# ChengeLi/LongTerm360FoV

Measured on AMD Instinct MI355X. Metric: sequences/sec (batch=1024, T_in=30->T_out=30, h=256), higher is better.
Workload: dtype f32; 1 GPU; configs[1]: target-only seq2seq inference (encoder + autoregressive decoder), H=256, batch=1024 per GPU, T_in=30->T_out=30, F_enc=90, F_dec=6, fp32, act=sigmoid, impl=auto; global_batch=1024, parallelism=replicas x1 (no collective)

## Files before the change

include/fov360.h:

```cpp
#ifndef FOV360_H
#define FOV360_H

#include <stddef.h>
#include <stdint.h>

#ifdef __cplusplus
extern "C" {
#endif

typedef void* fov_stream_t;

enum { FOV_ACT_SIGMOID = 0, FOV_ACT_HARD_SIGMOID = 1 };

enum {
    FOV_IMPL_AUTO = 0,
    FOV_IMPL_GENERIC = 1,
    FOV_IMPL_CLUSTER = 2
};

enum {
    FOV_OK = 0,
    FOV_ERR_INVALID = -1,
    FOV_ERR_UNSUPPORTED = -2,
    FOV_ERR_WORKSPACE = -3,
// ... 147 lines not shown
int fov_lstm_seq_fwd_zx(const float* zx, const float* R, const float* b, const float* h0, const float* c0,
                        float* hs, float* hT, float* cT, float* reserve,
                        int B, int T, int H, int act, int impl,
                        void* workspace, size_t workspace_bytes, fov_stream_t stream);

size_t fov_seq2seq_decode_workspace_bytes(int B, int T_in, int T_out, int F_enc, int F_dec, int H, int impl);
int fov_seq2seq_decode_fwd(const float* enc_in, const float* dec_in0,
                           const float* enc_K, const float* enc_R, const float* enc_b,
                           const float* dec_K, const float* dec_R, const float* dec_b,
                           const float* dense_W, const float* dense_b,
                           float* out, float* hT, float* cT,
                           int B, int T_in, int T_out, int F_enc, int F_dec, int H,
                           int act, int impl,
                           void* workspace, size_t workspace_bytes, fov_stream_t stream);

int fov_seq2seq_decoder_fwd(const float* dec_in0, const float* h0, const float* c0, const float* dec_K,
                            const float* dec_R, const float* dec_b, const float* dense_W, const float* dense_b,
                            float* out, float* hT, float* cT, int B, int T_out, int F_dec, int H, int act, int impl,
                            void* workspace, size_t workspace_bytes, fov_stream_t stream);

int fov_stacked_seq2seq_decode_supported(int B, int T_in, int T_out, int F_enc, int F_dec, int H, int L);
int fov_stacked_seq2seq_decode_fwd(const float* enc_in, const float* dec_in0,
                                   const float* enc0_K, const float* enc0_R, const float* enc0_b,
                                   const float* enc1_K, const float* enc1_R, const float* enc1_b,
                                   const float* enc2_K, const float* enc2_R, const float* enc2_b,
                                   const float* dec0_K, const float* dec0_R, const float* dec0_b,
                                   const float* dec1_K, const float* dec1_R, const float* dec1_b,
                                   const float* dec2_K, const float* dec2_R, const float* dec2_b,
                                   const float* dense_W, const float* dense_b,
                                   float* out, float* hT, float* cT,
// ... 249 lines not shown
```

longterm360fov_amd/_lib.py:

```python
import ctypes
import os

_HERE = os.path.dirname(os.path.abspath(__file__))
LIB_PATH = os.environ.get("FOV_LIB_PATH") or os.path.join(_HERE, "lib", "libfov360_hip.so")

ACT_SIGMOID = 0
ACT_HARD_SIGMOID = 1
IMPL_AUTO = 0
IMPL_GENERIC = 1
IMPL_CLUSTER = 2

OK = 0
ERR_INVALID = -1
ERR_UNSUPPORTED = -2
ERR_WORKSPACE = -3
ERR_LAUNCH = -4
ERR_TIMEOUT = -5

_P = ctypes.c_void_p
_I = ctypes.c_int
_SZ = ctypes.c_size_t

SIGNATURES = {
    "fov_last_error": (ctypes.c_char_p, []),
# ... 7 lines not shown
    "fov_mix_head_bwd": (_I, [_P] * 9 + [_I] * 3 + [_P]),
    "fov_mix_decoder_workspace_bytes": (_SZ, [_I] * 2),
    "fov_mix_decoder_fwd": (_I, [_P] * 6 + [ctypes.c_int64] * 2 + [_P] * 21 + [_I] * 5 + [_P, _SZ, _P]),
    "fov_mix_decoder_fwd_bf16": (_I, [_P] * 6 + [ctypes.c_int64] * 2 + [_P] * 21 + [_I] * 5 + [_P, _SZ, _P]),
    "fov_lstm_seq_fwd_bf16": (_I, [_P] * 10 + [_I] * 5 + [_P, _SZ, _P]),
    "fov_seq2seq_decode_fwd_bf16": (_I, [_P] * 13 + [_I] * 7 + [_P, _SZ, _P]),
    "fov_dense_fwd_bf16": (_I, [_P] * 4 + [_I] * 4 + [_P]),
    "fov_mix_decoder_bwd_workspace_bytes": (_SZ, [_I] * 2),
    "fov_mix_decoder_bwd": (_I, [_P] * 21 + [_I] * 5 + [_P, _SZ, _P]),
    "fov_mix_decoder_bwd_bf16": (_I, [_P] * 21 + [_I] * 5 + [_P, _SZ, _P]),
    "fov_matmul_workspace_bytes": (_SZ, [_I] * 3),
    "fov_matmul": (_I, [_P] * 3 + [_I] * 3 + [_P, _SZ, _P]),
    "fov_lstm_seq_fwd_zx": (_I, [_P] * 9 + [_I] * 5 + [_P, _SZ, _P]),
    "fov_seq2seq_decode_workspace_bytes": (_SZ, [_I] * 7),
    "fov_seq2seq_decode_fwd": (_I, [_P] * 13 + [_I] * 8 + [_P, _SZ, _P]),
    "fov_seq2seq_decoder_fwd": (_I, [_P] * 11 + [_I] * 6 + [_P, _SZ, _P]),
    "fov_stacked_seq2seq_decode_supported": (_I, [_I] * 7),
    "fov_stacked_seq2seq_decode_fwd": (_I, [_P] * 25 + [_I] * 8 + [_P]),
    "fov_selffed_decoder_supported": (_I, [_I] * 4),
    "fov_selffed_decoder_fwd": (_I, [_P] * 15 + [_I] * 6 + [_P]),
    "fov_selffed_decoder_bwd": (_I, [_P] * 14 + [_I] * 7 + [_P]),
    "fov_stacked_seq2seq_train_supported": (_I, [_I] * 7),
    "fov_stacked_seq2seq_train_bwd_scratch_bytes": (_SZ, [_I] * 4),
    "fov_stacked_seq2seq_train_fwd": (_I, [_P] * 15 + [_I] * 8 + [_P]),
    "fov_stacked_seq2seq_train_bwd": (_I, [_P] * 10 + [_I] * 6 + [_P, _SZ, _P]),
    "fov_seq2seq_tf_workspace_bytes": (_SZ, [_I] * 7),
    "fov_seq2seq_tf_fwd": (_I, [_P] * 11 + [_I] * 8 + [_P, _SZ, _P]),
    "fov_meanvar_xyz": (_I, [_P, _P, ctypes.c_int64, _I, _P]),
    "fov_lstm_seq_fwd_train": (_I, [_P] * 10 + [_I] * 6 + [_P, _SZ, _P]),
    "fov_lstm_seq_bwd_workspace_bytes": (_SZ, [_I] * 4),
# ... 127 lines not shown
```

longterm360fov_amd/csrc/api_lstm.hip:

```cpp
#include "fov_common.h"
#include "xch_common.h"
#include "bf16_common.h"

namespace fov {

static bool want_cluster(int impl, int F, int H, int F_dec, bool decode) {
    if (impl == FOV_IMPL_GENERIC) return false;
    const bool ok = cluster_shape_ok(F, H) && (!decode || (F_dec >= 1 && F_dec <= 8)) && device_cu_count() >= H / 64;
    return impl == FOV_IMPL_CLUSTER ? true : ok;
}

static LstmParams layer_params(const float* x, const float* K, const float* R, const float* b, const float* h0, const float* c0,
                               float* hs, float* hT, float* cT, float* reserve, int B, int T, int F, int H, int act, void* workspace) {
    LstmParams p = {};
    p.x = x; p.K = K; p.R = R; p.b = b; p.h0 = h0; p.c0 = c0; p.hs = hs; p.hT = hT; p.cT = cT; p.reserve = reserve;
    p.B = B; p.T = T; p.F = F; p.H = H; p.act = act;
    bind_workspace(p, workspace);
    return p;
}

enum class FwdKernel { Wide16, Wide512, Wide, Cluster, Stepwise, Generic };
struct FwdPlan {
    FwdKernel kernel;
    size_t need;
// ... 400 lines not shown

int fov_mix_decoder_bwd_bf16(const float* M, const float* P, const float* dloss, const float* res1, const float* res2,
                             const float* C1, const float* C2, const float* dec1_K, const float* dec1_R, const float* dec2_K,
                             const float* dec2_R, const float* dense_W, const float* mix_Wp, float* DZ1, float* DZ2,
                             float* dpre_m, float* dpre_p, float* dh1_0, float* dc1_0, float* dh2_0, float* dc2_0, int B,
                             int T_out, int H, int O, int act, void* workspace, size_t workspace_bytes, fov_stream_t stream) {
    return mix_decoder_bwd_impl(M, P, dloss, res1, res2, C1, C2, dec1_K, dec1_R, dec2_K, dec2_R, dense_W, mix_Wp, DZ1, DZ2, dpre_m,
                                dpre_p, dh1_0, dc1_0, dh2_0, dc2_0, B, T_out, H, O, act, workspace, workspace_bytes, stream, true);
}

size_t fov_seq2seq_decode_workspace_bytes(int B, int T_in, int T_out, int F_enc, int F_dec, int H, int impl) {
    (void)T_in;
    return plan_decode(B, T_out, F_enc, F_dec, H, impl).need;
}

int fov_seq2seq_decode_fwd(const float* enc_in, const float* dec_in0, const float* enc_K, const float* enc_R,
                           const float* enc_b, const float* dec_K, const float* dec_R, const float* dec_b,
                           const float* dense_W, const float* dense_b, float* out, float* hT, float* cT, int B,
                           int T_in, int T_out, int F_enc, int F_dec, int H, int act, int impl, void* workspace,
                           size_t workspace_bytes, fov_stream_t stream) {
    if (B < 0 || T_in < 0 || T_out < 0 || F_enc <= 0 || F_dec <= 0 || H <= 0 || !enc_K || !enc_R || !enc_b ||
        !dec_K || !dec_R || !dec_b || !dense_W || !dense_b ||
        (B > 0 && ((T_in > 0 && !enc_in) || !dec_in0 || (T_out > 0 && !out))) || !valid_act(act)) {
        set_error("fov_seq2seq_decode_fwd: invalid argument");
        return FOV_ERR_INVALID;
    }
    if (F_dec > 64) { set_error("fov_seq2seq_decode_fwd: F_dec > 64 unsupported"); return FOV_ERR_UNSUPPORTED; }
    const DecodePlan plan = plan_decode(B, T_out, F_enc, F_dec, H, impl);
    if (int rc = check_ws(workspace, workspace_bytes, plan.need)) return rc;
    LstmParams p = {};
    p.x = enc_in; p.K = enc_K; p.R = enc_R; p.b = enc_b; p.T = T_in; p.F = F_enc;
    bind_decoder(p, dec_in0, dec_K, dec_R, dec_b, dense_W, dense_b, out, hT, cT, B, T_out, F_dec, H, act, workspace);
    hipStream_t s = (hipStream_t)stream;
    switch (plan.kernel) {
        case DecodeKernel::Wide16: return launch_wide16_s2s(p, s);
        case DecodeKernel::Cluster: return launch_cluster(p, true, s);
        case DecodeKernel::Generic: break;
    }
    return launch_generic(p, true, s);
}

int fov_seq2seq_decoder_fwd(const float* dec_in0, const float* h0, const float* c0, const float* dec_K,
                            const float* dec_R, const float* dec_b, const float* dense_W, const float* dense_b, float* out,
                            float* hT, float* cT, int B, int T_out, int F_dec, int H, int act, int impl, void* workspace,
                            size_t workspace_bytes, fov_stream_t stream) {
    if (B < 0 || T_out < 0 || F_dec <= 0 || H <= 0 || !dec_K || !dec_R || !dec_b || !dense_W || !dense_b ||
        (B > 0 && (!dec_in0 || (T_out > 0 && !out))) || !valid_act(act)) {
        set_error("fov_seq2seq_decoder_fwd: invalid argument");
        return FOV_ERR_INVALID;
    }
    if (F_dec > 64) { set_error("fov_seq2seq_decoder_fwd: F_dec > 64 unsupported"); return FOV_ERR_UNSUPPORTED; }
    const DecodePlan plan = plan_decode(B, T_out, 1, F_dec, H, impl);
    if (int rc = check_ws(workspace, workspace_bytes, plan.need)) return rc;
    LstmParams p = {};
// ... 40 lines not shown
```

longterm360fov_amd/csrc/fov_common.h:

```cpp
#pragma once
#include <hip/hip_runtime.h>
#include <stdint.h>

#include "../../include/fov360.h"

namespace fov {

typedef float f32x4 __attribute__((ext_vector_type(4)));

__device__ __forceinline__ float sigmoid_f(float x) {
    return __builtin_amdgcn_rcpf(1.0f + __expf(-x));
}
__device__ __forceinline__ float hard_sigmoid_f(float x) {
    return fminf(fmaxf(fmaf(0.2f, x, 0.5f), 0.0f), 1.0f);
}
__device__ __forceinline__ float tanh_f(float x) {
    return 1.0f - 2.0f * __builtin_amdgcn_rcpf(1.0f + __expf(2.0f * x));
}
template <int ACT>
__device__ __forceinline__ float rec_act(float x) {
    return ACT == FOV_ACT_HARD_SIGMOID ? hard_sigmoid_f(x) : sigmoid_f(x);
}
template <int ACT>
__device__ __forceinline__ float rec_act_grad(float a) {
// ... 29 lines not shown
    const float* db;
    const float* dW;
    const float* dbias;
    float* out;
    int B, T, F, H;
    int T_out, F_dec;
    int act;
    unsigned long long* xch;
    unsigned* status;
    int num_groups;
    int num_tiles;
    int epoch_span;
    int force_safe_exchange;
    int xcd_pad;
    int trio;
};

int launch_generic(const LstmParams& p, bool decode, hipStream_t stream);
long generic_launch_count();
bool wide16_s2s_shape(int B, int F_enc, int F_dec, int H);
int launch_wide16_s2s(const LstmParams& p, hipStream_t stream);
int launch_cluster(const LstmParams& p, bool decode, hipStream_t stream);
int launch_cluster_decoder(const LstmParams& p, hipStream_t stream);
bool cluster_shape_ok(int F, int H);
bool stacked_s2s_shape_ok(int B, int T_in, int T_out, int F_enc, int F_dec, int H, int L);
bool selffed_shape_ok(int B, int T, int O, int H);
size_t cluster_workspace_bytes(int B, int H);
int cluster_num_groups(int B, int H);
int device_cu_count();
struct EnvKnobs {
    int force_safe_exchange, two_launches, resident_limit;
// ... 235 lines not shown
```

longterm360fov_amd/csrc/lstm_cluster.hip:

```cpp
#include <stdlib.h>

#include <atomic>
#include <mutex>

#include "fov_common.h"
#include "xch_common.h"

namespace fov {

constexpr int BT = 16;
constexpr int XR = 6;
constexpr int KPAD = 2;
constexpr int NXBUF = 3;
constexpr int CL_MAX_F = 96;
constexpr int CL_MAX_O = 8;

constexpr int MODE_LAYER = 0;
constexpr int MODE_DECODE = 1;
constexpr int MODE_LAYER_ZX = 2;

typedef unsigned u32x2 __attribute__((ext_vector_type(2)));
typedef unsigned u32x4g __attribute__((ext_vector_type(4)));
typedef float f32x2 __attribute__((ext_vector_type(2)));
template <bool V> struct BoolC { static constexpr bool value = V; };
// ... 141 lines not shown
template <int H>
__device__ __forceinline__ void load_r_block(float (&wR)[H / 16][4][4], int j, const float* R, int col0, int slice, int lane) {
    constexpr int G = H / 64;
    const int n = lane & 15, g4 = lane >> 4;
    const int H4 = 4 * H;
    const __amdgpu_buffer_rsrc_t rrs = __builtin_amdgcn_make_buffer_rsrc(const_cast<float*>(R), 0, H * H4 * 4, 0x00020000);
    const unsigned voff = (unsigned)((4 * g4 * H4 + col0 + n) * 4);
    const unsigned kb = (unsigned)((((slice + (j >> 2)) & (G - 1)) * 64 + (j & 3) * 16) * H4 * 4);
#pragma unroll
    for (int s = 0; s < 4; ++s)
#pragma unroll
        for (int g = 0; g < 4; ++g)
            wR[j][s][g] = __uint_as_float(__builtin_amdgcn_raw_buffer_load_b32(rrs, voff, kb + (unsigned)((s * H4 + g * H) * 4), 0));
}
template <int H>
__device__ __forceinline__ void load_dec_small(float (&bias)[4], f32x4 (&kb)[2], const float* K, const float* b, int F, int col0, int lane) {
    const int n = lane & 15, g4 = lane >> 4;
    const int H4 = 4 * H;
    const __amdgpu_buffer_rsrc_t brs = __builtin_amdgcn_make_buffer_rsrc(const_cast<float*>(b), 0, b ? H4 * 4 : 0, 0x00020000);
#pragma unroll
    for (int g = 0; g < 4; ++g) bias[g] = __uint_as_float(__builtin_amdgcn_raw_buffer_load_b32(brs, (unsigned)((g * H + col0 + n) * 4), 0, 0));
    const __amdgpu_buffer_rsrc_t krs = __builtin_amdgcn_make_buffer_rsrc(const_cast<float*>(K), 0, F * H4 * 4, 0x00020000);
#pragma unroll
    for (int s = 0; s < 2; ++s) {
        const unsigned voff = (unsigned)(((4 * s + g4) * H4 + col0 + n) * 4);
#pragma unroll
        for (int g = 0; g < 4; ++g) kb[s][g] = __uint_as_float(__builtin_amdgcn_raw_buffer_load_b32(krs, voff + (unsigned)(g * H * 4), 0, 0));
    }
}

// ... 98 lines not shown
            for (int g = 0; g < 4; ++g) {
                if (CINIT && j == J0 && s == 0) mfma_f32_c<true>(acc[g], a[s], wR[j][s][g], c0[g], false);
                else mfma_f32<true>(acc[g], a[s], wR[j][s][g], mf_pos(FIRST && !CINIT, LAST, j == J0 && s == 0, j == J1 - 1 && s == 3 && g == 3));
            }
        a = an;
    }
}

struct ClusterCarry {
    unsigned epoch;
    XchTicket ticket;
    bool same_xcd, aborted, xch_used;
    float c[4], h[4];
};

template <int H, int ACT, int MODE, int FUSED>
__device__ __forceinline__ void cluster_body(const LstmParams& p, ClusterCarry& cy) {
    constexpr int G = H / 64;
    constexpr int NQ = H / 16;
    constexpr int NG = (G - 1) * 2;
    constexpr bool LAYER = (MODE != MODE_DECODE);
    constexpr bool ZX = (MODE == MODE_LAYER_ZX);
    constexpr bool F1 = (FUSED == 1), F2 = (FUSED == 2);
    constexpr bool FZ = (FUSED != 0);
    extern __shared__ __attribute__((aligned(16))) float smem[];

    const int tid = threadIdx.x, lane = tid & 63, wave = tid >> 6;
    const int n = lane & 15, g4 = lane >> 4;
    constexpr unsigned OORB = 0x80000000u;
#ifdef FOV_STAMPS
    if (blockIdx.x == 5 && tid == 0) g_stamps[MODE & 1][STAMP_STEPS - 1][0] = __builtin_amdgcn_s_memtime();
#endif
// ... 8 lines not shown
        __syncthreads();
    }
    int group, slice;
    if (G > 1 && ((p.num_groups & 7) == 0 || p.xcd_pad)) {
        group = (blockIdx.x / (8 * G)) * 8 + (blockIdx.x & 7);
        slice = (blockIdx.x >> 3) & (G - 1);
    } else {
        group = blockIdx.x / G;
        slice = blockIdx.x - group * G;
    }
    const int col0 = slice * 64 + wave * 16;

    const float* Kp = LAYER ? p.K : p.dK;
    const float* Rp = LAYER ? p.R : p.dR;
    const float* bp = LAYER ? p.b : p.db;
    const int F = LAYER ? (ZX ? 0 : p.F) : p.F_dec;
    const int steps = LAYER ? p.T : p.T_out;
    const int Fp = round16(F);
    const int nq = Fp >> 4;

    const ClusterLds L = cluster_lds(H, F, !LAYER);
    const int LDX = L.ldx, LDH = L.ldh;
    float* sK = smem + L.off_k;
    float* sH = smem + L.off_h;
    float* sX = smem + L.off_x;
    float* sY = smem + L.off_w;
    int* sFlag = (int*)(smem + L.off_flag);
    float* sKw = sK + wave * (nq * 4 + KPAD) * 256;

    const bool xch_used = (G > 1) && (!LAYER || p.T > 1 || F1);
    unsigned* sXch = (unsigned*)(sFlag + 4);
    const bool hdr = xch_used && !F2;
    unsigned hdr_base = 0, hdr_launch = 0;
    if (hdr && tid == 0) {
        hdr_base = xch_status_load(p.status + ST_EPOCH);
        hdr_launch = xch_status_load(p.status + ST_LAUNCHES);
    }
    float wR[NQ][4][4];
    float bias[4];
    constexpr int JA = NQ < 3 ? NQ : 3;
    constexpr int STREAM_LA = 3;
    f32x4 kb[2];
    if constexpr (F2) {
        load_dec_small<H>(bias, kb, Kp, bp, F, col0, lane);
    } else {
        load_weights<H, !LAYER, 0, JA, false>(wR, bias, sKw, Kp, Rp, bp, F, Fp, col0, slice, lane);
    }
    unsigned long long* hello = p.xch + (size_t)p.num_groups * 2 * BT * H + (size_t)group * G;
    const unsigned my_xcc = xcc_id();
    if (hdr && tid == 0) {
        sXch[0] = hdr_base;
        sXch[1] = hdr_launch;
        st_granule(hello + slice, (((unsigned long long)hdr_base + 1ull) << 32) | my_xcc);
        xch_count_arrival(p.status);
    }
    FOV_PSTAMP(3);
    if constexpr (!F2) load_weights<H, !LAYER, JA, NQ, true>(wR, bias, sKw, Kp, Rp, bp, F, Fp, col0, slice, lane);
    FOV_PSTAMP(2);
    const bool poisoned = hdr && xch_poisoned(p.status);
    if (tid == 0) { sFlag[0] = (poisoned || (F2 && cy.aborted)) ? 1 : 0; sFlag[1] = 0; }
    if (hdr && !poisoned && tid < G) {
        const unsigned long long hello_tag = (unsigned long long)sXch[0] + 1ull;
        unsigned long long hv = 0;
        unsigned spins = 0;
        while (true) {
            hv = ld_granule(hello + tid);
            if ((hv >> 32) == hello_tag) break;
            if (xch_wait_expired(++spins, p.status)) {
                xch_give_up(p.status);
                sFlag[0] = 1;
                break;
            }
// ... 23 lines not shown
    float bd4[4];
    if (!LAYER) {
        const int O = p.F_dec;
        const __amdgpu_buffer_rsrc_t wdrs = __builtin_amdgcn_make_buffer_rsrc(const_cast<float*>(p.dW), 0, H * O * 4, 0x00020000);
        const __amdgpu_buffer_rsrc_t bdrs = __builtin_amdgcn_make_buffer_rsrc(const_cast<float*>(p.dbias), 0, O * 4, 0x00020000);
#pragma unroll
        for (int ss = 0; ss < 4; ++ss) {
            const int unit = col0 + 4 * g4 + ss;
            const int o = 4 * (n & 3) + (n >> 2);
            wd[ss] = __uint_as_float(__builtin_amdgcn_raw_buffer_load_b32(wdrs, (o < O) ? (unsigned)((unit * O + o) * 4) : OORB, 0, 0));
        }
#pragma unroll
        for (int ss = 0; ss < 4; ++ss)
            bd4[ss] = __uint_as_float(__builtin_amdgcn_raw_buffer_load_b32(bdrs, (4 * ss + g4 < O) ? (unsigned)((4 * ss + g4) * 4) : OORB, 0, 0));
    }
    if constexpr (F2) {
#pragma unroll
        for (int j = 0; j < STREAM_LA; ++j) load_r_block<H>(wR, j, Rp, col0, slice, lane);
    } else if (!LAYER) {
        __syncthreads();
        kb[0] = *(const f32x4*)(sKw + lane * 4);
        kb[1] = *(const f32x4*)(sKw + 256 + lane * 4);
    }

    __syncthreads();
    FOV_PSTAMP(5);
    XchTicket ticket = {0u, 0u, false};
    if (xch_used && !F2) ticket = xch_ticket(sXch);
    if constexpr (F2) ticket = cy.ticket;
    unsigned epoch = F2 ? cy.epoch : ticket.base;
    const bool same_xcd = F2 ? cy.same_xcd : (xch_used && (sFlag[1] == 0) && (p.force_safe_exchange == 0));
    bool aborted = F2 ? cy.aborted : (xch_used && sFlag[0] != 0);
    if (xch_used && !F2 && tid == 0 && !same_xcd && !aborted)
// ... 97 lines not shown
#pragma unroll
            for (int tt = 0; tt < 2; ++tt)
                if (tt < steps) {
#pragma unroll
                    for (int i = 0; i < XR; ++i)
                        if (xcl + 16 * i < F) xl[tt * BT * LDX + 16 * i] = x2[tt][i];
                }
        }
        const __amdgpu_buffer_rsrc_t yors = __builtin_amdgcn_make_buffer_rsrc(
            (!LAYER && p.out) ? p.out + (size_t)b0 * p.T_out * p.F_dec : nullptr, 0, (!LAYER && p.out) ? live_rows * p.T_out * p.F_dec * 4 : 0, 0x00020000);
        unsigned yoff[2];
#pragma unroll
        for (int ss = 0; ss < 2; ++ss)
            yoff[ss] = (!LAYER && 4 * ss + g4 < p.F_dec && (!F2 || (slice == 0 && wave == 0))) ? (unsigned)((n * p.T_out * p.F_dec + 4 * ss + g4) * 4) : OORB;
        f32x4 y4 = (f32x4){0.f, 0.f, 0.f, 0.f};
        if (!LAYER) {
            const __amdgpu_buffer_rsrc_t y0rs = __builtin_amdgcn_make_buffer_rsrc(
                const_cast<float*>(p.dec_in0 + (size_t)b0 * F), 0, live_rows * F * 4, 0x00020000);
#pragma unroll
            for (int ss = 0; ss < 4; ++ss)
                y4[ss] = __uint_as_float(__builtin_amdgcn_raw_buffer_load_b32(y0rs, (4 * ss + g4 < F) ? (unsigned)((n * F + 4 * ss + g4) * 4) : OORB, 0, 0));
        }
        __syncthreads();
        FOV_PSTAMP(6);

        f32x4 bias4[4];
#pragma unroll
        for (int g = 0; g < 4; ++g) bias4[g] = (f32x4){bias[g], bias[g], bias[g], bias[g]};
        asm volatile("" : "+v"(bias4[0]), "+v"(bias4[1]), "+v"(bias4[2]), "+v"(bias4[3]));
        f32x4 acc[4];
#pragma unroll
        for (int g = 0; g < 4; ++g) acc[g] = bias4[g];
        if (ZX && steps > 0) {
#pragma unroll
            for (int g = 0; g < 4; ++g)
#pragma unroll
                for (int r = 0; r < 4; ++r)
                    acc[g][r] = bias[g] + __uint_as_float(__builtin_amdgcn_raw_buffer_load_b32(zxrs, zxoff + (unsigned)((r * p.T * 4 * H + g * H) * 4), 0, 0));
        }
        if (steps > 0) {
            if constexpr (ZX) input_proj_any<true, true>(acc, sX + n * LDX + 4 * g4, sKw, nq, lane);
            else if constexpr (LAYER) input_proj_any<true, true, true>(acc, sX + n * LDX + 4 * g4, sKw, nq, lane, bias4);
            else input_proj_reg<true, true>(acc, y4, kb, bias4);
            if constexpr (F2) {
                f32x4 a = *(const f32x4*)hrow;
#pragma unroll
                for (int j = 0; j < NQ; ++j) {
                    if (j + STREAM_LA < NQ) load_r_block<H>(wR, j + STREAM_LA, Rp, col0, slice, lane);
                    f32x4 an = a;
                    if (j + 1 < NQ) an = *(const f32x4*)(hrow + 16 * (j + 1));
#pragma unroll
                    for (int s2 = 0; s2 < 4; ++s2)
#pragma unroll
                        for (int g = 0; g < 4; ++g)
                            mfma_f32<true>(acc[g], a[s2], wR[j][s2][g], mf_pos(false, true, false, j == NQ - 1 && s2 == 3 && g == 3));
                    a = an;
                }
            } else if (!h_zero) {
                recurrent<H, 0, 4, true, true>(acc, hrow, wR);
            }
        }

        float xr[XR];
// ... 317 lines not shown
}

template <int H, int ACT, int MODE>
__global__ __launch_bounds__(256, 1) void lstm_cluster_kernel(LstmParams p) {
    if constexpr (H >= 128) {
        if (p.xcd_pad && (int)((blockIdx.x / (8 * (H / 64))) * 8 + (blockIdx.x & 7)) >= p.num_groups) {
            const bool exchanging = (MODE == MODE_DECODE) || p.T > 1;
            if (threadIdx.x == 0 && exchanging) xch_count_arrival(p.status);
            return;
        }
    }
    ClusterCarry cy;
    cluster_body<H, ACT, MODE, 0>(p, cy);
}

template <int H, int ACT>
__global__ __launch_bounds__(256, 1) void lstm_cluster_fused_kernel(LstmParams p) {
    if constexpr (H >= 128) {
        if (p.xcd_pad && (int)((blockIdx.x / (8 * (H / 64))) * 8 + (blockIdx.x & 7)) >= p.num_groups) {
            if (threadIdx.x == 0) xch_count_arrival(p.status);
            return;
        }
    }
    ClusterCarry cy;
    cluster_body<H, ACT, MODE_LAYER, 1>(p, cy);
    cluster_body<H, ACT, MODE_DECODE, 2>(p, cy);
}

int device_cu_count() {
    static std::atomic<int> cus[64];
    int dev = 0, n = 256;
    if (hipGetDevice(&dev) == hipSuccess && dev >= 0 && dev < 64 && (n = cus[dev].load(std::memory_order_relaxed)) == 0) {
        hipDeviceProp_t prop;
        n = (hipGetDeviceProperties(&prop, dev) == hipSuccess && prop.multiProcessorCount > 0) ? prop.multiProcessorCount : 256;
        cus[dev].store(n, std::memory_order_relaxed);
    }
    const int lim = env_knobs().resident_limit;
    return (lim > 0 && lim < n) ? lim : n;
}

int ensure_dynamic_lds(const void* kern, size_t lds, int block) {
// ... 61 lines not shown
        set_error("cluster kernel: H=%d F=%d needs %zu B of LDS (> 160 KiB)", H, F, lds);
        return FOV_ERR_UNSUPPORTED;
    }
    int rc = ensure_dynamic_lds((const void*)kern, lds);
    if (rc) return rc;
    LstmParams q = p;
    const int padded = xch_padded_groups(q.num_groups);
    q.xcd_pad = (H >= 128 && !env_knobs().no_xcd_pad && (q.num_groups & 7) != 0 && device_cu_count() >= padded * (H / 64)) ? 1 : 0;
    const dim3 grid((q.xcd_pad ? padded : q.num_groups) * (H / 64)), block(256);
    hipLaunchKernelGGL(kern, grid, block, lds, stream, q);
    return launch_check("cluster");
}

template <int H>
static int launch_cluster_fused_h(const LstmParams& p, hipStream_t stream) {
    void (*kern)(LstmParams) = p.act == FOV_ACT_HARD_SIGMOID ? lstm_cluster_fused_kernel<H, FOV_ACT_HARD_SIGMOID>
                                                             : lstm_cluster_fused_kernel<H, FOV_ACT_SIGMOID>;
    const ClusterLds L1 = cluster_lds(H, p.F, false), L2 = cluster_lds(H, p.F_dec, true);
    const size_t lds = (size_t)(L1.total_floats > L2.total_floats ? L1.total_floats : L2.total_floats) * sizeof(float);
    if (lds > 160 * 1024) { set_error("fused cluster kernel: needs %zu B of LDS (> 160 KiB)", lds); return FOV_ERR_UNSUPPORTED; }
    int rc = ensure_dynamic_lds((const void*)kern, lds);
    if (rc) return rc;
    LstmParams q = p;
    const bool no_pad = env_knobs().no_xcd_pad != 0;
    const int padded = (q.num_groups + 7) & ~7;
    q.xcd_pad = (H >= 128 && !no_pad && (q.num_groups & 7) != 0 && device_cu_count() >= padded * (H / 64)) ? 1 : 0;
    hipLaunchKernelGGL(kern, dim3((q.xcd_pad ? padded : q.num_groups) * (H / 64)), dim3(256), lds, stream, q);
    return launch_check("fused cluster");
}

static int launch_cluster_fused(const LstmParams& p, hipStream_t stream) {
    switch (p.H) {
// ... 81 lines not shown
```

longterm360fov_amd/ops.py:

```python
import os

import torch

from . import _lib
from ._lib import (ACT_HARD_SIGMOID, ACT_SIGMOID, IMPL_AUTO, IMPL_CLUSTER, IMPL_GENERIC,
                   FovError, check)

_ACT = {"sigmoid": ACT_SIGMOID, "hard_sigmoid": ACT_HARD_SIGMOID, ACT_SIGMOID: ACT_SIGMOID,
        ACT_HARD_SIGMOID: ACT_HARD_SIGMOID}
_IMPL = {"auto": IMPL_AUTO, "generic": IMPL_GENERIC, "cluster": IMPL_CLUSTER, IMPL_AUTO: IMPL_AUTO,
         IMPL_GENERIC: IMPL_GENERIC, IMPL_CLUSTER: IMPL_CLUSTER}


def act_code(act):
    return _ACT[act]


def impl_code(impl):
    return _IMPL[impl]


def _dev(t, name):
    if t is None:
        return None
# ... 14 lines not shown
    if _raw_stream is not None and _raw_device is not None:
        return _raw_stream(_raw_device())
    return torch.cuda.current_stream().cuda_stream


_ENV_KNOBS = ("FOV_FORCE_SAFE_EXCHANGE", "FOV_TWO_LAUNCHES", "FOV_DBG_RESIDENT_LIMIT", "FOV_NO_CELL_PATCH", "FOV_NO_CONV_PATCH", "FOV_NO_WIDE16", "FOV_BWD_STEPPED",
              "FOV_NO_WGRAD_FUSION", "FOV_NO_DX_FUSION", "FOV_BWD_GROUPS4", "FOV_GEMM_BF16_NOREMAP", "FOV_GEMM_BF16_SPLIT", "FOV_GEMM_BF16_SHALLOW", "FOV_NO_WGRAD_GROUP", "FOV_NO_WIDE16_TRIO", "FOV_DBG_TRACE", "FOV_GEMM_VARIANT",
              "FOV_GEMM_SPLIT", "FOV_NO_XCD_PAD", "FOV_XCD_PAD_MAX", "FOV_NO_BWD16_NARROW", "FOV_BWD16_GROUPS", "FOV_NO_STACK2", "FOV_NO_WGRAD_LINES", "FOV_NO_WGRAD_BF16_TILES", "FOV_NO_STACKED_DECODE",
              "FOV_NO_SELFFED_FUSED", "FOV_NO_STACKED_TRAIN")
_env_seen = None
_ENV_DATA = getattr(os.environ, "_data", None)
_ENV_KEYS_B = tuple(os.fsencode(k) for k in _ENV_KNOBS)
if not isinstance(_ENV_DATA, dict) or (_ENV_DATA and not isinstance(next(iter(_ENV_DATA)), bytes)):
    _ENV_DATA = None
_FORCE_SAFE_KEY_B = os.fsencode("FOV_FORCE_SAFE_EXCHANGE")


def _env_snapshot():
    if _ENV_DATA is not None:
        return tuple(map(_ENV_DATA.get, _ENV_KEYS_B))
    return tuple(os.environ.get(k) for k in _ENV_KNOBS)


def _sync_env():
    global _env_seen
    cur = _env_snapshot()
    if cur != _env_seen:
        if _env_seen is not None or any(v is not None for v in cur):
            _lib.lib().fov_reload_env()
        _env_seen = cur
# ... 9 lines not shown
        holder._forced = (holder.buf.data_ptr(), want)


def _new_workspace(nbytes, device):
    buf = torch.empty(nbytes + 256, dtype=torch.uint8, device=device)
    with torch.cuda.device(buf.device):
        check(_lib.lib().fov_workspace_init(buf.data_ptr(), buf.numel(), _stream()))
    return buf


class Workspace:

    def __init__(self, device=None):
        self.device = device
        self.buf = None

    def get(self, nbytes, device):
        nbytes = max(int(nbytes), 256)
        if self.buf is None or self.buf.numel() < nbytes or self.buf.device != device:
            self.buf = _new_workspace(nbytes, device)
        _apply_force_safe(self)
        return self.buf

    def check(self):
        if self.buf is not None:
            check(_lib.lib().fov_check_status(self.buf.data_ptr(), self.buf.numel(), _stream()))


    def exchange_mode(self):
        return _lib.lib().fov_exchange_mode(self.buf.data_ptr(), self.buf.numel(), _stream())
# ... 72 lines not shown
    H = ws_t[1].shape[0]
    F_dec = ws_t[6].shape[1]
    assert dec_in0.shape == (B, 1, F_dec)
    if out is None:
        out = torch.empty((B, T_out, F_dec), dtype=torch.float32, device=enc_in.device)
    L = _lib.lib()
    ws = (workspace or default_workspace(enc_in.device))
    if dtype == "bf16":
        buf = ws.get(L.fov_lstm_seq_workspace_bytes(B, T_in, 128, 256, IMPL_CLUSTER), enc_in.device)
        check(L.fov_seq2seq_decode_fwd_bf16(_ptr(enc_in), _ptr(dec_in0), *[_ptr(t) for t in ws_t], _ptr(out),
                                            None if hT is None else _ptr(_dev(hT, "hT")), None if cT is None else _ptr(_dev(cT, "cT")),
                                            B, T_in, T_out, F_enc, F_dec, H, act_code(act), buf.data_ptr(), buf.numel(), _stream()))
        return out
    impl = impl_code(impl)
    buf = ws.get(L.fov_seq2seq_decode_workspace_bytes(B, T_in, T_out, F_enc, F_dec, H, impl), enc_in.device)
    check(L.fov_seq2seq_decode_fwd(_ptr(enc_in), _ptr(dec_in0), *[_ptr(t) for t in ws_t], _ptr(out),
                                   None if hT is None else _ptr(_dev(hT, "hT")), None if cT is None else _ptr(_dev(cT, "cT")),
                                   B, T_in, T_out, F_enc, F_dec, H, act_code(act), impl,
                                   buf.data_ptr(), buf.numel(), _stream()))
    return out


def seq2seq_decoder(dec_in0, h0, c0, w, T_out, act="sigmoid", impl="auto", workspace=None, out=None):
    dec_in0, h0, c0 = _dev(dec_in0, "dec_in0"), _dev(h0, "h0"), _dev(c0, "c0")
    ws_t = [_dev(w[k], k) for k in _W_ORDER[3:]]
    B, H = h0.shape
    F_dec = ws_t[3].shape[1]
    assert dec_in0.shape == (B, 1, F_dec)
    if out is None:
        out = torch.empty((B, T_out, F_dec), dtype=torch.float32, device=h0.device)
    L = _lib.lib()
    impl = impl_code(impl)
    ws = (workspace or default_workspace(h0.device))
    buf = ws.get(L.fov_seq2seq_decode_workspace_bytes(B, 0, T_out, 1, F_dec, H, impl), h0.device)
# ... 640 lines not shown
    check(L.fov_dense_mse_head(_ptr(hs), _ptr(W), _ptr(b), _ptr(target), None if y is None else _ptr(y), None if dx is None else _ptr(dx),
                               _ptr(_dev(dW, "dW")), _ptr(_dev(db, "db")), _ptr(loss), N, H, O, 1 if activation == "tanh" else 0, float(weight),
                               buf.data_ptr(), buf.numel(), _stream()))
    return y, dx, loss


def rmsprop_tf_step(params, grads, ms, lr, decay=0.9, eps=1e-10, clip_value=0.0, guards=None, applied=None):
    for t in (params, grads, ms):
        _dev(t, "flat buffer")
    if guards is None and applied is None:
        check(_lib.lib().fov_rmsprop_tf_step(_ptr(params), _ptr(grads), _ptr(ms), params.numel(), lr, decay, eps, clip_value,
                                             _stream()))
    else:
        check(_lib.lib().fov_rmsprop_tf_step_guarded(_ptr(params), _ptr(grads), _ptr(ms), params.numel(), lr, decay, eps, clip_value,
                                                     *_guard_ptrs(guards), _applied_ptr(applied), _stream()))


def dense_bwd(x, W, dpre, dW=None, db=None, need_dx=True, accumulate=False, scratch=None, need_dW=True, need_db=True,
              dtype="f32"):
    x, W, dpre = _dev(x, "x"), _dev(W, "W"), _dev(dpre, "dpre")
    In, Out = W.shape
    x2, d2 = x.reshape(-1, In), dpre.reshape(-1, Out)
    N = x2.shape[0]
    e = lambda *s: torch.empty(s, dtype=torch.float32, device=x.device)
    dW = (e(In, Out) if dW is None else dW) if need_dW else None
    db = (e(Out) if db is None else db) if need_db else None
    dx = e(N, In) if need_dx else None
    L = _lib.lib()
    buf = (scratch or _default_scratch).get(L.fov_dense_bwd_workspace_bytes(N, In, Out), x.device)
    fn = L.fov_dense_bwd_bf16 if dtype == "bf16" else L.fov_dense_bwd
# ... 77 lines not shown
    return out


def _applied_ptr(applied):
    if applied is None:
        return None
    assert applied.is_cuda and applied.dtype == torch.int64 and applied.numel() == 1
    return applied.data_ptr()


def adam_step(params, grads, m, v, step, lr=1e-3, beta1=0.9, beta2=0.999, eps=1e-7, guards=None, applied=None):
    for t in (params, grads, m, v):
        _dev(t, "flat buffer")
    check(_lib.lib().fov_adam_step_guarded(_ptr(params), _ptr(grads), _ptr(m), _ptr(v), params.numel(), lr, beta1, beta2,
                                           eps, int(step), *_guard_ptrs(guards), _applied_ptr(applied), _stream()))


def reduce_defer_begin(grad, arena):
    check(_lib.lib().fov_reduce_defer_begin(_ptr(grad), grad.numel(), arena.data_ptr(), arena.numel() * arena.element_size(), _stream()))


def reduce_defer_flush(grad=None):
    check(_lib.lib().fov_reduce_defer_flush(None if grad is None else _ptr(grad), _stream()))


def reduce_defer_end(grad=None):
    check(_lib.lib().fov_reduce_defer_end(None if grad is None else _ptr(grad), _stream()))


def rmsprop_step(params, grads, accum, lr=1e-3, rho=0.9, eps=1e-7, guards=None, applied=None):
    for t in (params, grads, accum):
        _dev(t, "flat buffer")
    check(_lib.lib().fov_rmsprop_step_guarded(_ptr(params), _ptr(grads), _ptr(accum), params.numel(), lr, rho, eps,
                                              *_guard_ptrs(guards), _applied_ptr(applied), _stream()))


def matmul(a, b, scratch=None):
    a, b = _dev(a, "a"), _dev(b, "b")
    M, K = a.shape
    N = b.shape[1]
    c = torch.empty((M, N), dtype=torch.float32, device=a.device)
    L = _lib.lib()
    buf = (scratch or _default_scratch).get(min(L.fov_matmul_workspace_bytes(M, K, N), 64 << 20), a.device)
    check(L.fov_matmul(_ptr(a), _ptr(b), _ptr(c), M, K, N, buf.data_ptr(), buf.numel(), _stream()))
    return c


def dense_add(x, W, b, add, activation="tanh", out=None):
    x, W = _dev(x, "x"), _dev(W, "W")
# ... 582 lines not shown
```

Baseline: 3.158 million sequences/s.

## Prepack recurrent LSTM weights into a lane-contiguous layout for vector loads

Adds a kernel that repacks each recurrent weight matrix R so that every lane's 4x4 block is contiguous. The fused cluster kernel can then fetch each block with 128-bit buffer loads instead of scalar ones, and it deepens the R streaming lookahead when the pack is present. It also prefetches the decoder's first input before the step loop. On the Python side, the pack is built after a couple of calls with the same weight tensor and cached, keyed by pointer and version. Optimizer steps now bump the parameter version so a stale pack is not reused, at the cost of extra memory and a more complex invalidation path.

After: 3.191 million sequences/s (median of 6 runs). 1.01x the previous value.

```diff
diff --git a/include/fov360.h b/include/fov360.h
--- a/include/fov360.h
+++ b/include/fov360.h
@@ -185,6 +185,18 @@
                            int act, int impl,
                            void* workspace, size_t workspace_bytes, fov_stream_t stream);
 
+int fov_lstm_pack_r(const float* R, int H, float* out, fov_stream_t stream);
+
+int fov_seq2seq_decode_fwd_packed(const float* enc_in, const float* dec_in0,
+                                  const float* enc_K, const float* enc_R, const float* enc_b,
+                                  const float* dec_K, const float* dec_R, const float* dec_b,
+                                  const float* dense_W, const float* dense_b,
+                                  float* out, float* hT, float* cT,
+                                  const float* enc_Rpack, const float* dec_Rpack,
+                                  int B, int T_in, int T_out, int F_enc, int F_dec, int H,
+                                  int act, int impl,
+                                  void* workspace, size_t workspace_bytes, fov_stream_t stream);
+
 int fov_seq2seq_decoder_fwd(const float* dec_in0, const float* h0, const float* c0, const float* dec_K,
                             const float* dec_R, const float* dec_b, const float* dense_W, const float* dense_b,
                             float* out, float* hT, float* cT, int B, int T_out, int F_dec, int H, int act, int impl,
diff --git a/longterm360fov_amd/_lib.py b/longterm360fov_amd/_lib.py
--- a/longterm360fov_amd/_lib.py
+++ b/longterm360fov_amd/_lib.py
@@ -45,6 +45,8 @@
     "fov_lstm_seq_fwd_zx": (_I, [_P] * 9 + [_I] * 5 + [_P, _SZ, _P]),
     "fov_seq2seq_decode_workspace_bytes": (_SZ, [_I] * 7),
     "fov_seq2seq_decode_fwd": (_I, [_P] * 13 + [_I] * 8 + [_P, _SZ, _P]),
+    "fov_lstm_pack_r": (_I, [_P, _I, _P, _P]),
+    "fov_seq2seq_decode_fwd_packed": (_I, [_P] * 15 + [_I] * 8 + [_P, _SZ, _P]),
     "fov_seq2seq_decoder_fwd": (_I, [_P] * 11 + [_I] * 6 + [_P, _SZ, _P]),
     "fov_stacked_seq2seq_decode_supported": (_I, [_I] * 7),
     "fov_stacked_seq2seq_decode_fwd": (_I, [_P] * 25 + [_I] * 8 + [_P]),
diff --git a/longterm360fov_amd/csrc/api_lstm.hip b/longterm360fov_amd/csrc/api_lstm.hip
--- a/longterm360fov_amd/csrc/api_lstm.hip
+++ b/longterm360fov_amd/csrc/api_lstm.hip
@@ -438,15 +438,20 @@
     return plan_decode(B, T_out, F_enc, F_dec, H, impl).need;
 }
 
-int fov_seq2seq_decode_fwd(const float* enc_in, const float* dec_in0, const float* enc_K, const float* enc_R,
-                           const float* enc_b, const float* dec_K, const float* dec_R, const float* dec_b,
-                           const float* dense_W, const float* dense_b, float* out, float* hT, float* cT, int B,
-                           int T_in, int T_out, int F_enc, int F_dec, int H, int act, int impl, void* workspace,
-                           size_t workspace_bytes, fov_stream_t stream) {
+static int seq2seq_decode_fwd_impl(const float* enc_in, const float* dec_in0, const float* enc_K, const float* enc_R,
+                                   const float* enc_b, const float* dec_K, const float* dec_R, const float* dec_b,
+                                   const float* dense_W, const float* dense_b, float* out, float* hT, float* cT,
+                                   const float* enc_Rpack, const float* dec_Rpack, int B, int T_in, int T_out, int F_enc,
+                                   int F_dec, int H, int act, int impl, void* workspace, size_t workspace_bytes,
+                                   fov_stream_t stream) {
     if (B < 0 || T_in < 0 || T_out < 0 || F_enc <= 0 || F_dec <= 0 || H <= 0 || !enc_K || !enc_R || !enc_b ||
         !dec_K || !dec_R || !dec_b || !dense_W || !dense_b ||
         (B > 0 && ((T_in > 0 && !enc_in) || !dec_in0 || (T_out > 0 && !out))) || !valid_act(act)) {
         set_error("fov_seq2seq_decode_fwd: invalid argument");
+        return FOV_ERR_INVALID;
+    }
+    if ((((uintptr_t)enc_Rpack | (uintptr_t)dec_Rpack) & 15) != 0) {
+        set_error("fov_seq2seq_decode_fwd_packed: a pack must be 16-byte aligned");
         return FOV_ERR_INVALID;
     }
     if (F_dec > 64) { set_error("fov_seq2seq_decode_fwd: F_dec > 64 unsupported"); return FOV_ERR_UNSUPPORTED; }
@@ -455,6 +460,7 @@
     LstmParams p = {};
     p.x = enc_in; p.K = enc_K; p.R = enc_R; p.b = enc_b; p.T = T_in; p.F = F_enc;
     bind_decoder(p, dec_in0, dec_K, dec_R, dec_b, dense_W, dense_b, out, hT, cT, B, T_out, F_dec, H, act, workspace);
+    if (lstm_pack_shape_ok(H)) { p.Rpack = enc_Rpack; p.dRpack = dec_Rpack; }
     hipStream_t s = (hipStream_t)stream;
     switch (plan.kernel) {
         case DecodeKernel::Wide16: return launch_wide16_s2s(p, s);
@@ -462,6 +468,26 @@
         case DecodeKernel::Generic: break;
     }
     return launch_generic(p, true, s);
+}
+
+int fov_seq2seq_decode_fwd(const float* enc_in, const float* dec_in0, const float* enc_K, const float* enc_R,
+                           const float* enc_b, const float* dec_K, const float* dec_R, const float* dec_b,
+                           const float* dense_W, const float* dense_b, float* out, float* hT, float* cT, int B,
+                           int T_in, int T_out, int F_enc, int F_dec, int H, int act, int impl, void* workspace,
+                           size_t workspace_bytes, fov_stream_t stream) {
+    return seq2seq_decode_fwd_impl(enc_in, dec_in0, enc_K, enc_R, enc_b, dec_K, dec_R, dec_b, dense_W, dense_b, out, hT, cT,
+                                   nullptr, nullptr, B, T_in, T_out, F_enc, F_dec, H, act, impl, workspace, workspace_bytes, stream);
+}
+
+int fov_seq2seq_decode_fwd_packed(const float* enc_in, const float* dec_in0, const float* enc_K, const float* enc_R,
+                                  const float* enc_b, const float* dec_K, const float* dec_R, const float* dec_b,
+                                  const float* dense_W, const float* dense_b, float* out, float* hT, float* cT,
+                                  const float* enc_Rpack, const float* dec_Rpack, int B, int T_in, int T_out, int F_enc,
+                                  int F_dec, int H, int act, int impl, void* workspace, size_t workspace_bytes,
+                                  fov_stream_t stream) {
+    return seq2seq_decode_fwd_impl(enc_in, dec_in0, enc_K, enc_R, enc_b, dec_K, dec_R, dec_b, dense_W, dense_b, out, hT, cT,
+                                   enc_Rpack, dec_Rpack, B, T_in, T_out, F_enc, F_dec, H, act, impl, workspace, workspace_bytes,
+                                   stream);
 }
 
 int fov_seq2seq_decoder_fwd(const float* dec_in0, const float* h0, const float* c0, const float* dec_K,
diff --git a/longterm360fov_amd/csrc/fov_common.h b/longterm360fov_amd/csrc/fov_common.h
--- a/longterm360fov_amd/csrc/fov_common.h
+++ b/longterm360fov_amd/csrc/fov_common.h
@@ -67,7 +67,11 @@
     int force_safe_exchange;
     int xcd_pad;
     int trio;
-};
+    const float* Rpack;
+    const float* dRpack;
+};
+bool lstm_pack_shape_ok(int H);
+int launch_lstm_pack_r(const float* R, int H, float* out, hipStream_t stream);
 
 int launch_generic(const LstmParams& p, bool decode, hipStream_t stream);
 long generic_launch_count();
diff --git a/longterm360fov_amd/csrc/lstm_cluster.hip b/longterm360fov_amd/csrc/lstm_cluster.hip
--- a/longterm360fov_amd/csrc/lstm_cluster.hip
+++ b/longterm360fov_amd/csrc/lstm_cluster.hip
@@ -179,6 +179,24 @@
             wR[j][s][g] = __uint_as_float(__builtin_amdgcn_raw_buffer_load_b32(rrs, voff, kb + (unsigned)((s * H4 + g * H) * 4), 0));
 }
 template <int H>
+__device__ __forceinline__ void load_r_block_packed(float (&wR)[H / 16][4][4], int j, const float* Rpack, int col0, int slice, int lane) {
+    constexpr int G = H / 64, NQ = H / 16;
+    const __amdgpu_buffer_rsrc_t rrs = __builtin_amdgcn_make_buffer_rsrc(const_cast<float*>(Rpack), 0, H * 4 * H * 4, 0x00020000);
+    const unsigned voff = (unsigned)((col0 >> 4) * NQ * 4096 + lane * 16);
+    const unsigned kb = (unsigned)((((slice + (j >> 2)) & (G - 1)) * 4 + (j & 3)) * 4096);
+#pragma unroll
+    for (int s = 0; s < 4; ++s) {
+        const u32x4g v = __builtin_amdgcn_raw_buffer_load_b128(rrs, voff, kb + (unsigned)(s * 1024), 0);
+#pragma unroll
+        for (int g = 0; g < 4; ++g) wR[j][s][g] = __uint_as_float(v[g]);
+    }
+}
+template <int H, int J0, int J1>
+__device__ __forceinline__ void load_r_packed(float (&wR)[H / 16][4][4], const float* Rpack, int col0, int slice, int lane) {
+#pragma unroll
+    for (int j = J0; j < J1; ++j) load_r_block_packed<H>(wR, j, Rpack, col0, slice, lane);
+}
+template <int H>
 __device__ __forceinline__ void load_dec_small(float (&bias)[4], f32x4 (&kb)[2], const float* K, const float* b, int F, int col0, int lane) {
     const int n = lane & 15, g4 = lane >> 4;
     const int H4 = 4 * H;
@@ -307,8 +325,9 @@
     float c[4], h[4];
 };
 
-template <int H, int ACT, int MODE, int FUSED>
+template <int H, int ACT, int MODE, int FUSED, bool PK = false>
 __device__ __forceinline__ void cluster_body(const LstmParams& p, ClusterCarry& cy) {
+    static_assert(!PK || FUSED != 0, "the pack is read by the fused kernel only");
     constexpr int G = H / 64;
     constexpr int NQ = H / 16;
     constexpr int NG = (G - 1) * 2;
@@ -347,6 +366,7 @@
     const float* Kp = LAYER ? p.K : p.dK;
     const float* Rp = LAYER ? p.R : p.dR;
     const float* bp = LAYER ? p.b : p.db;
+    const float* Rpk = LAYER ? p.Rpack : p.dRpack;
     const int F = LAYER ? (ZX ? 0 : p.F) : p.F_dec;
     const int steps = LAYER ? p.T : p.T_out;
     const int Fp = round16(F);
@@ -372,10 +392,13 @@
     float wR[NQ][4][4];
     float bias[4];
     constexpr int JA = NQ < 3 ? NQ : 3;
-    constexpr int STREAM_LA = 3;
+    constexpr int F2_SMALL_LOADS = 4 + 8 + 4 + 4 + 4;
+    constexpr int STREAM_LA = !PK ? 3 : ((63 - F2_SMALL_LOADS) / 4 < NQ ? (63 - F2_SMALL_LOADS) / 4 : NQ);
     f32x4 kb[2];
     if constexpr (F2) {
         load_dec_small<H>(bias, kb, Kp, bp, F, col0, lane);
+    } else if constexpr (PK) {
+        load_r_packed<H, 0, JA>(wR, Rpk, col0, slice, lane);
     } else {
         load_weights<H, !LAYER, 0, JA, false>(wR, bias, sKw, Kp, Rp, bp, F, Fp, col0, slice, lane);
     }
@@ -388,7 +411,12 @@
         xch_count_arrival(p.status);
     }
     FOV_PSTAMP(3);
-    if constexpr (!F2) load_weights<H, !LAYER, JA, NQ, true>(wR, bias, sKw, Kp, Rp, bp, F, Fp, col0, slice, lane);
+    if constexpr (PK && !F2) {
+        load_r_packed<H, JA, NQ>(wR, Rpk, col0, slice, lane);
+        load_weights<H, !LAYER, NQ, NQ, true>(wR, bias, sKw, Kp, Rp, bp, F, Fp, col0, slice, lane);
+    } else if constexpr (!F2) {
+        load_weights<H, !LAYER, JA, NQ, true>(wR, bias, sKw, Kp, Rp, bp, F, Fp, col0, slice, lane);
+    }
     FOV_PSTAMP(2);
     const bool poisoned = hdr && xch_poisoned(p.status);
     if (tid == 0) { sFlag[0] = (poisoned || (F2 && cy.aborted)) ? 1 : 0; sFlag[1] = 0; }
@@ -442,9 +470,22 @@
         for (int ss = 0; ss < 4; ++ss)
             bd4[ss] = __uint_as_float(__builtin_amdgcn_raw_buffer_load_b32(bdrs, (4 * ss + g4 < O) ? (unsigned)((4 * ss + g4) * 4) : OORB, 0, 0));
     }
+    float y0pre[4] = {0.f, 0.f, 0.f, 0.f};
+    if constexpr (F2 && PK) {
+        const int b00 = group * BT;
+        const int live0 = p.B - b00 < BT ? p.B - b00 : BT;
+        const __amdgpu_buffer_rsrc_t y0rs = __builtin_amdgcn_make_buffer_rsrc(
+            const_cast<float*>(p.dec_in0 + (size_t)b00 * F), 0, live0 > 0 ? live0 * F * 4 : 0, 0x00020000);
+#pragma unroll
+        for (int ss = 0; ss < 4; ++ss)
+            y0pre[ss] = __uint_as_float(__builtin_amdgcn_raw_buffer_load_b32(y0rs, (4 * ss + g4 < F) ? (unsigned)((n * F + 4 * ss + g4) * 4) : OORB, 0, 0));
+    }
     if constexpr (F2) {
 #pragma unroll
-        for (int j = 0; j < STREAM_LA; ++j) load_r_block<H>(wR, j, Rp, col0, slice, lane);
+        for (int j = 0; j < STREAM_LA; ++j) {
+            if constexpr (PK) load_r_block_packed<H>(wR, j, Rpk, col0, slice, lane);
+            else load_r_block<H>(wR, j, Rp, col0, slice, lane);
+        }
     } else if (!LAYER) {
         __syncthreads();
         kb[0] = *(const f32x4*)(sKw + lane * 4);
@@ -572,7 +613,10 @@
         for (int ss = 0; ss < 2; ++ss)
             yoff[ss] = (!LAYER && 4 * ss + g4 < p.F_dec && (!F2 || (slice == 0 && wave == 0))) ? (unsigned)((n * p.T_out * p.F_dec + 4 * ss + g4) * 4) : OORB;
         f32x4 y4 = (f32x4){0.f, 0.f, 0.f, 0.f};
-        if (!LAYER) {
+        if constexpr (F2 && PK) {
+#pragma unroll
+            for (int ss = 0; ss < 4; ++ss) y4[ss] = y0pre[ss];
+        } else if (!LAYER) {
             const __amdgpu_buffer_rsrc_t y0rs = __builtin_amdgcn_make_buffer_rsrc(
                 const_cast<float*>(p.dec_in0 + (size_t)b0 * F), 0, live_rows * F * 4, 0x00020000);
 #pragma unroll
@@ -596,7 +640,7 @@
                 for (int r = 0; r < 4; ++r)
                     acc[g][r] = bias[g] + __uint_as_float(__builtin_amdgcn_raw_buffer_load_b32(zxrs, zxoff + (unsigned)((r * p.T * 4 * H + g * H) * 4), 0, 0));
         }
-        if (steps > 0) {
+        if ((F2 && PK) || steps > 0) {
             if constexpr (ZX) input_proj_any<true, true>(acc, sX + n * LDX + 4 * g4, sKw, nq, lane);
             else if constexpr (LAYER) input_proj_any<true, true, true>(acc, sX + n * LDX + 4 * g4, sKw, nq, lane, bias4);
             else input_proj_reg<true, true>(acc, y4, kb, bias4);
@@ -604,7 +648,10 @@
                 f32x4 a = *(const f32x4*)hrow;
 #pragma unroll
                 for (int j = 0; j < NQ; ++j) {
-                    if (j + STREAM_LA < NQ) load_r_block<H>(wR, j + STREAM_LA, Rp, col0, slice, lane);
+                    if (j + STREAM_LA < NQ) {
+                        if constexpr (PK) load_r_block_packed<H>(wR, j + STREAM_LA, Rpk, col0, slice, lane);
+                        else load_r_block<H>(wR, j + STREAM_LA, Rp, col0, slice, lane);
+                    }
                     f32x4 an = a;
                     if (j + 1 < NQ) an = *(const f32x4*)(hrow + 16 * (j + 1));
 #pragma unroll
@@ -952,7 +999,7 @@
     cluster_body<H, ACT, MODE, 0>(p, cy);
 }
 
-template <int H, int ACT>
+template <int H, int ACT, bool PK>
 __global__ __launch_bounds__(256, 1) void lstm_cluster_fused_kernel(LstmParams p) {
     if constexpr (H >= 128) {
         if (p.xcd_pad && (int)((blockIdx.x / (8 * (H / 64))) * 8 + (blockIdx.x & 7)) >= p.num_groups) {
@@ -961,8 +1008,8 @@
         }
     }
     ClusterCarry cy;
-    cluster_body<H, ACT, MODE_LAYER, 1>(p, cy);
-    cluster_body<H, ACT, MODE_DECODE, 2>(p, cy);
+    cluster_body<H, ACT, MODE_LAYER, 1, PK>(p, cy);
+    cluster_body<H, ACT, MODE_DECODE, 2, PK>(p, cy);
 }
 
 int device_cu_count() {
@@ -1054,8 +1101,10 @@
 
 template <int H>
 static int launch_cluster_fused_h(const LstmParams& p, hipStream_t stream) {
-    void (*kern)(LstmParams) = p.act == FOV_ACT_HARD_SIGMOID ? lstm_cluster_fused_kernel<H, FOV_ACT_HARD_SIGMOID>
-                                                             : lstm_cluster_fused_kernel<H, FOV_ACT_SIGMOID>;
+    const bool pk = p.Rpack && p.dRpack;
+    void (*kern)(LstmParams) = p.act == FOV_ACT_HARD_SIGMOID
+                                   ? (pk ? lstm_cluster_fused_kernel<H, FOV_ACT_HARD_SIGMOID, true> : lstm_cluster_fused_kernel<H, FOV_ACT_HARD_SIGMOID, false>)
+                                   : (pk ? lstm_cluster_fused_kernel<H, FOV_ACT_SIGMOID, true> : lstm_cluster_fused_kernel<H, FOV_ACT_SIGMOID, false>);
     const ClusterLds L1 = cluster_lds(H, p.F, false), L2 = cluster_lds(H, p.F_dec, true);
     const size_t lds = (size_t)(L1.total_floats > L2.total_floats ? L1.total_floats : L2.total_floats) * sizeof(float);
     if (lds > 160 * 1024) { set_error("fused cluster kernel: needs %zu B of LDS (> 160 KiB)", lds); return FOV_ERR_UNSUPPORTED; }
diff --git a/longterm360fov_amd/csrc/lstm_pack.hip b/longterm360fov_amd/csrc/lstm_pack.hip
--- /dev/null
+++ b/longterm360fov_amd/csrc/lstm_pack.hip
@@ -0,0 +1,40 @@
+#include "fov_common.h"
+
+namespace fov {
+
+template <int H>
+__global__ __launch_bounds__(256) void lstm_pack_r_kernel(const float* __restrict__ R, float* __restrict__ out) {
+    constexpr int NQ = H / 16;
+    const int t = blockIdx.x * 256 + threadIdx.x;
+    const int lane = t & 63, s = (t >> 6) & 3, blk = t >> 8;
+    const int jj = blk % NQ, c = blk / NQ;
+    const int n = lane & 15, g4 = lane >> 4;
+    const float* src = R + (size_t)(16 * jj + 4 * g4 + s) * (4 * H) + 16 * c + n;
+    f32x4 v;
+#pragma unroll
+    for (int g = 0; g < 4; ++g) v[g] = src[g * H];
+    *(f32x4*)(out + (size_t)t * 4) = v;
+}
+
+bool lstm_pack_shape_ok(int H) { return H == 64 || H == 128 || H == 256; }
+
+int launch_lstm_pack_r(const float* R, int H, float* out, hipStream_t stream) {
+    const dim3 grid(H * H / 256), block(256);
+    switch (H) {
+        case 64: hipLaunchKernelGGL(lstm_pack_r_kernel<64>, grid, block, 0, stream, R, out); break;
+        case 128: hipLaunchKernelGGL(lstm_pack_r_kernel<128>, grid, block, 0, stream, R, out); break;
+        default: hipLaunchKernelGGL(lstm_pack_r_kernel<256>, grid, block, 0, stream, R, out); break;
+    }
+    return launch_check("lstm_pack_r");
+}
+
+}
+
+using namespace fov;
+
+extern "C" int fov_lstm_pack_r(const float* R, int H, float* out, fov_stream_t stream) {
+    if (!R || !out) { set_error("fov_lstm_pack_r: invalid argument"); return FOV_ERR_INVALID; }
+    if (!lstm_pack_shape_ok(H)) { set_error("fov_lstm_pack_r: H in {64, 128, 256} only (got %d)", H); return FOV_ERR_UNSUPPORTED; }
+    if (((uintptr_t)out & 15) != 0) { set_error("fov_lstm_pack_r: out must be 16-byte aligned"); return FOV_ERR_INVALID; }
+    return launch_lstm_pack_r(R, H, out, (hipStream_t)stream);
+}
diff --git a/longterm360fov_amd/ops.py b/longterm360fov_amd/ops.py
--- a/longterm360fov_amd/ops.py
+++ b/longterm360fov_amd/ops.py
@@ -52,6 +52,16 @@
 if not isinstance(_ENV_DATA, dict) or (_ENV_DATA and not isinstance(next(iter(_ENV_DATA)), bytes)):
     _ENV_DATA = None
 _FORCE_SAFE_KEY_B = os.fsencode("FOV_FORCE_SAFE_EXCHANGE")
+_NO_PACK_KEY_B = os.fsencode("FOV_NO_WEIGHT_PACK")
+_PACK_AFTER = 2
+_increment_version = getattr(getattr(torch.autograd, "graph", None), "increment_version", None)
+
+
+def _mark_written(t):
+    if _increment_version is not None:
+        _increment_version(t)
+    else:
+        t.add_(0)
 
 
 def _env_snapshot():
@@ -91,6 +101,26 @@
     def __init__(self, device=None):
         self.device = device
         self.buf = None
+        self._rpacks = {}
+
+    def r_pack(self, role, R):
+        no_pack = _ENV_DATA.get(_NO_PACK_KEY_B) == b"1" if _ENV_DATA is not None else os.environ.get("FOV_NO_WEIGHT_PACK", "") == "1"
+        H = R.shape[0]
+        if no_pack or H not in (64, 128, 256) or R.is_inference():
+            return None
+        key = (R.data_ptr(), R._version, R.shape, R.device)
+        e = self._rpacks.get(role)
+        if e is None or e[0] != key:
+            self._rpacks[role] = [key, R, 1, None]
+            return None
+        if e[3] is None:
+            e[2] += 1
+            if e[2] <= _PACK_AFTER:
+                return None
+            pack = torch.empty(H * 4 * H, dtype=torch.float32, device=R.device)
+            check(_lib.lib().fov_lstm_pack_r(R.data_ptr(), H, pack.data_ptr(), _stream()))
+            e[3] = pack
+        return e[3]
 
     def get(self, nbytes, device):
         nbytes = max(int(nbytes), 256)
@@ -193,10 +223,20 @@
         return out
     impl = impl_code(impl)
     buf = ws.get(L.fov_seq2seq_decode_workspace_bytes(B, T_in, T_out, F_enc, F_dec, H, impl), enc_in.device)
-    check(L.fov_seq2seq_decode_fwd(_ptr(enc_in), _ptr(dec_in0), *[_ptr(t) for t in ws_t], _ptr(out),
-                                   None if hT is None else _ptr(_dev(hT, "hT")), None if cT is None else _ptr(_dev(cT, "cT")),
-                                   B, T_in, T_out, F_enc, F_dec, H, act_code(act), impl,
-                                   buf.data_ptr(), buf.numel(), _stream()))
+    packs = (None, None)
+    if workspace is not None and impl != IMPL_GENERIC and B > 0:
+        packs = (workspace.r_pack("enc_R", ws_t[1]), workspace.r_pack("dec_R", ws_t[4]))
+    if packs[0] is None or packs[1] is None:
+        check(L.fov_seq2seq_decode_fwd(_ptr(enc_in), _ptr(dec_in0), *[_ptr(t) for t in ws_t], _ptr(out),
+                                       None if hT is None else _ptr(_dev(hT, "hT")), None if cT is None else _ptr(_dev(cT, "cT")),
+                                       B, T_in, T_out, F_enc, F_dec, H, act_code(act), impl,
+                                       buf.data_ptr(), buf.numel(), _stream()))
+    else:
+        check(L.fov_seq2seq_decode_fwd_packed(_ptr(enc_in), _ptr(dec_in0), *[_ptr(t) for t in ws_t], _ptr(out),
+                                              None if hT is None else _ptr(_dev(hT, "hT")), None if cT is None else _ptr(_dev(cT, "cT")),
+                                              packs[0].data_ptr(), packs[1].data_ptr(),
+                                              B, T_in, T_out, F_enc, F_dec, H, act_code(act), impl,
+                                              buf.data_ptr(), buf.numel(), _stream()))
     return out
 
 
@@ -867,6 +907,7 @@
     else:
         check(_lib.lib().fov_rmsprop_tf_step_guarded(_ptr(params), _ptr(grads), _ptr(ms), params.numel(), lr, decay, eps, clip_value,
                                                      *_guard_ptrs(guards), _applied_ptr(applied), _stream()))
+    _mark_written(params)
 
 
 def dense_bwd(x, W, dpre, dW=None, db=None, need_dx=True, accumulate=False, scratch=None, need_dW=True, need_db=True,
@@ -974,6 +1015,7 @@
         _dev(t, "flat buffer")
     check(_lib.lib().fov_adam_step_guarded(_ptr(params), _ptr(grads), _ptr(m), _ptr(v), params.numel(), lr, beta1, beta2,
                                            eps, int(step), *_guard_ptrs(guards), _applied_ptr(applied), _stream()))
+    _mark_written(params)
 
 
 def reduce_defer_begin(grad, arena):
@@ -993,6 +1035,7 @@
         _dev(t, "flat buffer")
     check(_lib.lib().fov_rmsprop_step_guarded(_ptr(params), _ptr(grads), _ptr(accum), params.numel(), lr, rho, eps,
                                               *_guard_ptrs(guards), _applied_ptr(applied), _stream()))
+    _mark_written(params)
 
 
 def matmul(a, b, scratch=None):
```
